# AngelAngelXie/Final-Project-Monte-Carlo-Path-Tracer-with-Microfacet-BSDF

Measured on AMD Instinct MI355X. Metric: Msamples/s (pixels x spp), chess scene 1920x1080, PSNR vs CPU, higher is better.
Workload: dtype f32

## Files before the change

### final-project-monte-carlo-path-tracer-with-microfacet-bsdf_amd/csrc/mcpt_frame.h

```cpp
#pragma once
#include "mcpt_host.h"
#include "mcpt_adaptive.h"
#include "mcpt_denoise.h"
#include "mcpt_temporal.h"

namespace mcpt {

constexpr int32_t kMaxAovSpp = 65536;

inline bool frame_ok(int W, int H) { return W > 0 && H > 0 && (uint64_t)W * H <= 0x7fffffffull / 8; }

enum : unsigned {
    kOneCallFrame = 1u,
    kOneRank = 2u,
    kDenoisedFrame = 4u,
    kOneSample = 8u
};

int check_frame_call(const char *name, const mcpt_camera &cam, const mcpt_params &p, unsigned forbid);

void fill_stats(mcpt_stats *stats, uint64_t samples, uint64_t traced_primary, int32_t n_dir, const Totals &rt, Clock::time_point t0);

struct FrameCall {
    mcpt_scene *sc;
    const mcpt_params &p;
    Clock::time_point t0;
    CameraConst cc;
    PixelSet ps;
    int begin(const mcpt_camera &cam) {
        HIP_TRY(hipSetDevice(sc->device));
        (void)hipGetLastError();
        t0 = Clock::now();
        cc = make_camera(cam);
        return MCPT_OK;
    }
    int pixels(int32_t spp, float spp_total, float *fb_dev, hipStream_t st) { return prepare_pixels(sc, cc, p, spp, spp_total, fb_dev, st, ps); }
    int end(mcpt_stats *stats, uint64_t samples, uint64_t traced_primary, const Totals &rt) const {
        if (stats) fill_stats(stats, samples, traced_primary, p.n_dir_sample, rt, t0);
        if (rt.overflow) return fail(MCPT_ERR_OVERFLOW, "some paths outran the clamp stack (raise params.max_depth)");
        return MCPT_OK;
    }
};

int aov_pass(mcpt_scene *sc, const CameraConst &cc, uint32_t seed, int32_t aov_spp, int32_t spec_depth, bool centre, float *aov_dev, hipStream_t st);
int check_features(const char *name, const mcpt_feature_opts *features, int32_t aov_spp, bool &centre);
int motion_pass(mcpt_scene *sc, const CameraConst &cc, const CameraConst &prev_cc, uint32_t seed, int32_t aov_spp, int32_t spec_depth, bool centre,
                float4 *maps, uint64_t map_rays, float *motion_dev, hipStream_t st);
uint64_t motion_map_rays(uint64_t n_px, int32_t aov_spp);

struct AdaptiveBufs {
    float *fb = nullptr;
    double *mom = nullptr;
    int32_t *spp = nullptr;
    float *err = nullptr;
    uint8_t *stamp = nullptr;
    const float *guide = nullptr;
    float guide_max_history = 0.f;
    uint32_t *list[2] = {nullptr, nullptr};
    int4 *cand[2] = {nullptr, nullptr};
    uint8_t *flags = nullptr;
    void *temp = nullptr;
// ... 59 lines not shown
```

### final-project-monte-carlo-path-tracer-with-microfacet-bsdf_amd/csrc/mcpt_host.h

```cpp
#pragma once
#include <hip/hip_runtime.h>

#include <algorithm>
#include <chrono>
#include <cstring>
#include <string>
#include <vector>

#include "mcpt_kernels.h"

namespace mcpt {

extern thread_local std::string g_err;

inline int fail(int code, const std::string &msg) {
    g_err = msg;
    return code;
}

#define HIP_TRY(expr)                                                                                   \
    do {                                                                                                \
        hipError_t e_ = (expr);                                                                         \
        if (e_ != hipSuccess)                                                                           \
            return fail(e_ == hipErrorOutOfMemory ? MCPT_ERR_OOM : MCPT_ERR_HIP,                        \
// ... 135 lines not shown
    DevBuf<int32_t> key_channel;
    int pix_key[5] = {0, 0, 0, 0, 0};
    uint32_t n_pix = 0;
};

struct Knobs {
    bool overlap = true;
    bool queue_ahead = true;
    bool timing = true;
    bool verbose = false;
    int pools = 1;
    int drain_batch = 4;
    uint64_t pool_min_work = 1ull << 20;
    uint32_t shadow_grid_per_cu = 128;
    uint32_t direct_grid_per_cu = 64;
    uint32_t ring_start = 0;
    int host_delay_us = 0;
    float halfspace_slack_scale = 1.f;
    float tir_bound_scale = 1.f;
    float cone_tol_scale = 1.f;
    float cull_rho_scale = 1.f;
    bool sky_cull = true;
    bool small_scene = true;
    uint64_t fake_free_mb = 0;
    void read();
};

enum KClass { K_CLOSEST = 0, K_SHADOW, K_SHADE, K_GENERATE, K_RESOLVE, K_DIRECT, K_NCLASS };

struct Timer {
    bool enabled = true;
    int bank = 0;
    std::vector<hipEvent_t> pool[2];
    struct Rec { int a, b, cls; };
    std::vector<Rec> recs[2];
    size_t used[2] = {0, 0};
    double ms[K_NCLASS] = {0, 0, 0, 0, 0, 0};
    uint64_t count[K_NCLASS] = {0, 0, 0, 0, 0, 0};
    Timer() = default;
    Timer(const Timer &) = delete;
    Timer &operator=(const Timer &) = delete;
    ~Timer() {
        for (int k = 0; k < 2; ++k)
            for (hipEvent_t e : pool[k]) (void)hipEventDestroy(e);
    }
    int get() {
// ... 16 lines not shown
        recs[bank].push_back({a, b, cls});
    }
    void collect_bank(int k) {
        for (const Rec &r : recs[k]) {
            float t = 0.f;
            if (hipEventElapsedTime(&t, pool[k][r.a], pool[k][r.b]) == hipSuccess) ms[r.cls] += t;
        }
        recs[k].clear();
        used[k] = 0;
    }
    void collect() {
        collect_bank(0);
        collect_bank(1);
    }
    void reset() {
        for (int i = 0; i < K_NCLASS; ++i) { ms[i] = 0; count[i] = 0; }
        for (int k = 0; k < 2; ++k) { recs[k].clear(); used[k] = 0; }
        bank = 0;
    }
};

struct Totals {
    uint64_t iterations = 0, shaded = 0, closest = 0, shadow = 0, direct = 0, pushes = 0, overflow = 0;
    double ms[K_NCLASS] = {0, 0, 0, 0, 0, 0};
    uint64_t cnt[K_NCLASS] = {0, 0, 0, 0, 0, 0};
    Totals &operator+=(const Totals &o) {
        iterations += o.iterations;
        shaded += o.shaded;
        closest += o.closest;
        shadow += o.shadow;
        direct += o.direct;
        pushes += o.pushes;
        overflow += o.overflow;
        for (int c = 0; c < K_NCLASS; ++c) {
            ms[c] += o.ms[c];
            cnt[c] += o.cnt[c];
        }
        return *this;
    }
};

struct GeomBufs {
    DevBuf<Node> nodes;
    DevBuf<QNode> qnodes;
    DevBuf<TriGeom> tri_geom;
    DevBuf<TriShade> tri_shade;
    DevBuf<SphereRec> spheres;
    DevBuf<mcpt_triangle> tris;
    DevBuf<LightRec> lights;
    DevBuf<LightNode> light_nodes;
    DevBuf<LightTri> light_tris;
    void swap_prims(GeomBufs &o) {
        nodes.swap(o.nodes);
        qnodes.swap(o.qnodes);
        tri_geom.swap(o.tri_geom);
        tri_shade.swap(o.tri_shade);
// ... 26 lines not shown
    BuildChoice choice;
};

struct alignas(16) MoveSeg {
    int32_t first_lane;
    int32_t count;
    int32_t first_tri;
    int32_t object;
    float m[12];
    float c0[3];
    int32_t raw;
};
static_assert(sizeof(MoveSeg) == 80, "MoveSeg must be 80 bytes");
void launch_move_objects(const MoveSeg *d_segs, int32_t n_segs, int32_t n_lanes, const mcpt_triangle *tris0, mcpt_triangle *tris_cur,
                         TriGeom *tri_geom, TriShade *tri_shade, SphereRec *spheres, hipStream_t s);

}

struct mcpt_scene {
    int device = 0;
    int device_sharers = 1;
    mcpt::Knobs knobs;
    mcpt_scene_info info{};
    mcpt::SceneMeta meta;
    mcpt::SceneSource src;
    mcpt::GeomBufs geom;
    mcpt::DevBuf<mcpt::TriGeom> snap_tri;
    mcpt::DevBuf<mcpt::SphereRec> snap_sph;
    bool has_snapshot = false;
    mcpt::DevBuf<mcpt_triangle> tris0;
    mcpt::DevBuf<int32_t> sphere_obj;
    mcpt::DevBuf<mcpt::MoveSeg> segs;
    mcpt::DevBuf<mcpt::MaterialRec> mats;
    mcpt::DevBuf<mcpt::InstRec> inst;
    mcpt::DevBuf<float> env;
    mcpt::DevBuf<unsigned long long> dbg;
    mcpt::DevScene view{};
    mcpt::Event fork;
    mcpt::SharedBufs shared;
    struct PoolCtx {
        mcpt::Stream main;
        mcpt::Stream side[2];
        mcpt::Event join[2];
        mcpt::Event book;
        mcpt::Event shaded, readback;
        int rc = 0;
// ... 67 lines not shown
```

### final-project-monte-carlo-path-tracer-with-microfacet-bsdf_amd/csrc/mcpt_kernels.h

```cpp
#pragma once
#include <hip/hip_runtime.h>

#include <cstddef>

#include "mcpt_device.h"

namespace mcpt {

constexpr uint32_t kFresh = 1u << 16;
constexpr uint32_t kTerminate = 1u << 17;
constexpr uint32_t kInside = 1u << 18;
constexpr uint32_t kPassBit = 1u << 20;
constexpr uint32_t kNoDirect = 1u << 19;

struct alignas(128) HotCounter {
    uint32_t v;
    uint32_t pad[31];
};
constexpr uint32_t kShadowShards = 32;
__host__ __device__ inline uint32_t shadow_region(uint32_t capacity) {
    return (((capacity + 63u) / 64u + kShadowShards - 1u) / kShadowShards) * 64u;
}
struct Counters {
    HotCounter n_paths[2];
    HotCounter n_rays[2];
    HotCounter n_direct[2];
    HotCounter free_head, free_tail;
    HotCounter n_prays[2];
    HotCounter live[2];
    HotCounter pushes;
    HotCounter overflow;
    HotCounter ended;
    unsigned long long tot_shaded, tot_direct, tot_shadow, tot_cont, tot_iterations, tot_pushes, tot_ended;
    uint32_t last_shadow;
    HotCounter n_shadow[2][kShadowShards];
    HotCounter n_shadow_w[2][kShadowShards];
};
constexpr size_t kCountersHeadBytes = offsetof(Counters, n_shadow);

struct Wave {
    uint4 *rec0;
    float4 *rec1;
    float4 *ray_o;
    float4 *ray_d;
    uint4 *hit;
    float *contrib;
    uint2 *fresh;
};

struct Scratch {
    float4 *vtx0;
    float4 *vtx1;
    float4 *vtx2;
    uint32_t *vtx_j;
    float4 *shq_o;
    float4 *shq_d;
};

constexpr int32_t kCandNone = 0x7fffffff;
constexpr int32_t kCandTraverse = 0x7ffffffe;

struct RenderConst {
    float rr_rate, inv_rr;
    int32_t n_dir, enable_shadow;
    uint32_t seed;
    int32_t mode;
    const uint32_t *pixel_list;
    const int4 *pixel_cand;
    int32_t s_pass[2], sample_offset[2];
    int32_t s_pass_shift[2];
    const uint32_t *key_pixel, *key_sample;
    const int32_t *key_channel;
    int32_t max_depth;
    int32_t track_live;
    uint32_t pool;
    float4 *stack;
    float *result[2];
    uint32_t *free_slots;
    uint32_t free_mask;
    uint32_t ray_cap;
    Counters *counters;
};

struct CameraConst {
    int32_t width, height, use_dof;
    float scale, aspect, focal_distance, aperture_radius;
    float eye[3];
    float orient[9];
};

constexpr int kSmallNodes = 64, kSmallTris = 64, kSmallSphereSlots = 16;
constexpr int kSmallMats = 12, kSmallLights = 4, kSmallLightNodes = 8, kSmallLightTris = 8;
constexpr int kSmallStk = 8;

struct RetryList {
    uint32_t *count;
    uint32_t *done;
// ... 57 lines not shown
```

### final-project-monte-carlo-path-tracer-with-microfacet-bsdf_amd/csrc/mcpt_kernels.hip

```cpp
#include <algorithm>
#include <cfloat>
#include <cstdlib>

#include "mcpt_kernels.h"
#include "mcpt_traverse.h"

namespace mcpt {

namespace {

#ifndef MCPT_SHADE_BLOCK
#define MCPT_SHADE_BLOCK 512
#endif
constexpr int kShadeBlock = MCPT_SHADE_BLOCK;

constexpr int kMaxAlloc = 9;
constexpr int kMaxWaves = 16;
struct BlockAllocShared {
    uint32_t cnt[kMaxWaves][kMaxAlloc];
    uint32_t base[kMaxAlloc];
};

template <int N>
MCPT_DI void block_alloc_begin(BlockAllocShared &sh, const bool (&want)[N], const uint32_t (&mult)[N], uint32_t *const (&counter)[N],
                               const bool (&subtract)[N], uint32_t (&prefix)[N]) {
    static_assert(N <= kMaxAlloc, "too many allocation requests");
    const uint32_t n_waves = blockDim.x >> 6;
    const uint32_t lane = lane_id();
    const uint32_t wave = threadIdx.x >> 6;
#pragma unroll
    for (int k = 0; k < N; ++k) {
        const unsigned long long mask = __ballot(want[k]);
        prefix[k] = __builtin_amdgcn_mbcnt_hi((uint32_t)(mask >> 32), __builtin_amdgcn_mbcnt_lo((uint32_t)mask, 0u));
        if (lane == 0) sh.cnt[wave][k] = (uint32_t)__popcll(mask);
    }
    __syncthreads();
#pragma unroll
    for (int k = 0; k < N; ++k) {
        if (threadIdx.x == (unsigned)k) {
// ... 504 lines not shown
    camera_ray_from<true>(cam, (int)(m % (uint32_t)cam.width), (int)(m / (uint32_t)cam.width), u, pos, dir);
    o[j] = make_float4(pos.x, pos.y, pos.z, 0.f);
    d[j] = make_float4(dir.x, dir.y, dir.z, 0.f);
}

__global__ __launch_bounds__(kBlock) void k_init_free(uint32_t *free_slots, Counters *c, uint32_t pool, uint32_t start, uint32_t mask) {
    const uint32_t j = blockIdx.x * kBlock + threadIdx.x;
    if (j < pool) free_slots[(start + j) & mask] = j;
    if (j == 0) {
        c->n_paths[0].v = c->n_paths[1].v = 0;
        c->n_rays[0].v = c->n_rays[1].v = 0;
        c->free_head.v = start;
        c->free_tail.v = start + pool;
        c->n_prays[0].v = c->n_prays[1].v = 0;
        c->live[0].v = c->live[1].v = 0;
        for (uint32_t k = 0; k < kShadowShards; ++k) {
            c->n_shadow[0][k].v = c->n_shadow[1][k].v = 0;
            c->n_shadow_w[0][k].v = c->n_shadow_w[1][k].v = 0;
        }
        c->n_direct[0].v = c->n_direct[1].v = 0;
        c->pushes.v = 0;
        c->overflow.v = 0;
        c->ended.v = 0;
        c->last_shadow = 0;
        c->tot_shaded = c->tot_direct = c->tot_shadow = c->tot_cont = c->tot_iterations = c->tot_pushes = c->tot_ended = 0;
    }
}

MCPT_DI bool sample_light(const DevScene &S, const float u[4], f3 &x_l, f3 &n_l, f3 &emit, float &pdf, int32_t &prim) {
    float area_sum = S.light_area_sum;
    const float p = u[0] * area_sum;
    area_sum = 0.f;
    for (int k = 0; k < S.n_lights; ++k) {
        const LightRec L = S.lights[k];
        area_sum += L.area;
        if (p <= area_sum) {
            const MaterialRec &m = S.mats[L.mat];
            if (L.kind == MCPT_OBJ_MESH) {
                float pp = sqrtf(u[1]) * L.root_area;
                int32_t ref = L.root;
                while (ref >= 0) {
                    const LightNode N = S.light_nodes[ref];
                    if (pp < N.left_area) {
                        ref = N.left;
                    } else {
                        pp = pp - N.left_area;
                        ref = N.right;
                    }
// ... 270 lines not shown
    const bool past_gate = false;
    const bool zero_direct = do_shade && direct_is_zero(S, m, q, n, wo, inside, ch, &by_tir);
#else
    const bool by_tir = false, past_gate = false;
    const bool zero_direct = do_shade && direct_is_zero(S, m, q, n, wo, inside, ch);
#endif
#if defined(MCPT_TRAVERSAL_STATS) || defined(MCPT_CHECK_DIRECT_SKIP)
    bool behind = false;
    if (do_shade && S.n_lights > 0) {
        const f3 L = mk3(S.light_center[0], S.light_center[1], S.light_center[2]) - q;
        behind = dot(L, L) > S.light_radius * S.light_radius * 1.0201f && emitters_behind(S, n, L);
    }
#else
    const bool behind = false;
#endif
#ifdef MCPT_CHECK_DIRECT_SKIP
    const bool need_direct = do_shade;
#else
    const bool need_direct = do_shade && !zero_direct;
#endif

    const bool ends_here = do_shade && !has_cont && !need_direct;
    const bool done = finished || ends_here;
    const bool want[9] = {done, do_shade && !ends_here, has_cont, need_direct, pushed, overflow, done && C.track_live && pq == 0,
                          done && C.track_live && pq == 1, ends_here};
    const uint32_t mult[9] = {1u, 1u, 1u, 1u, 1u, 1u, 1u, 1u, 1u};
    uint32_t *const ctr[9] = {&C.counters->free_tail.v, &C.counters->n_paths[next_idx].v, &C.counters->n_rays[next_idx].v,
                              &C.counters->n_direct[next_idx].v, &C.counters->pushes.v, &C.counters->overflow.v,
                              &C.counters->live[0].v, &C.counters->live[1].v, &C.counters->ended.v};
    const bool sub[9] = {false, false, false, false, false, false, true, true, false};
    uint32_t prefix[9], idx[9];
#ifdef MCPT_TRAVERSAL_STATS
    const long long tb0 = clock64();
#endif
    block_alloc_begin<9>(sh, want, mult, ctr, sub, prefix);
#ifdef MCPT_TRAVERSAL_STATS
    const long long tb1 = clock64();
#endif

    float kr = 0.f, ev = 0.f, aw = 0.f, pd = 0.f;
    f3 p2 = mk3(0, 0, 0), wi = mk3(0, 0, 1);
    if (do_shade) {
        const f3 mfn = mat_sample(m, n, u0[0], u0[1]);
        kr = mat_fresnel(m, rd, mfn, ch);
        const bool isReflect = u0[3] < kr;
        if (isReflect) p2 = (dot(wo, mfn) < 0) ? (p - n * kEps) : (p + n * kEps);
        else p2 = (dot(wo, mfn) < 0) ? (p + n * kEps) : (p - n * kEps);
        if (has_cont) {
            wi = isReflect ? mat_reflect(wo, mfn) : mat_refract(m, rd, mfn, ch);
            if (m.isDirac) {
                ev = mat_eval(m, wi, wo, n, ch, uv, isReflect);
                aw = -1.f;
            } else {
                aw = fabsf(dot(wo, n));
                mat_eval_pdf_rough(m, wi, wo, n, ch, uv, isReflect, ev, pd);
            }
        }
    }

#ifdef MCPT_TRAVERSAL_STATS
    const long long tb2 = clock64();
#endif
    block_alloc_end<9>(sh, mult, prefix, idx);
#ifdef MCPT_TRAVERSAL_STATS
    if (S.dbg && lane_id() == 0) {
        const long long tb3 = clock64();
        atomicAdd(&S.dbg[20], (unsigned long long)(tb1 - tb0));
        atomicAdd(&S.dbg[21], (unsigned long long)(tb3 - tb2));
        atomicAdd(&S.dbg[22], (unsigned long long)(tb3 - t_wave0));
        atomicAdd(&S.dbg[23], 1ull);
    }
    if (S.dbg) {
        int nd = 0;
        for (int t = 0; t < 4; ++t) nd += __ballot(do_shade && m.type == t) != 0ull ? 1 : 0;
        const unsigned long long ms = __ballot(do_shade);
        if (lane_id() == 0) {
            atomicAdd(&S.dbg[24 + nd], 1ull);
            atomicAdd(&S.dbg[29], (unsigned long long)__popcll(ms));
        }
    }
#endif
    if (done) C.free_slots[idx[0] & C.free_mask] = slot;
    if (!do_shade) return;
    if (ends_here) {
        const float l_dir = inside ? (float)((1. - (double)kr) * (double)0.f) : kr * 0.f;
        (pq ? C.result[1] : C.result[0])[pid] = unwind(C, slot, depth, l_dir);
        return;
    }
    const uint32_t j = idx[1], rj = idx[2], dj = idx[3];

    if (need_direct) {
        Xs.vtx0[dj] = make_float4(q.x, q.y, q.z, uv.x);
        Xs.vtx1[dj] = make_float4(n.x, n.y, n.z, uv.y);
        Xs.vtx2[dj] = make_float4(wo.x, wo.y, wo.z, __uint_as_float((uint32_t)mat_id | ((uint32_t)ch << 16) | (inside ? (1u << 18) : 0u) |
                                                                    (zero_direct ? (1u << 19) : 0u) | (behind ? (1u << 20) : 0u) | (by_tir ? (1u << 21) : 0u) |
                                                                    (past_gate ? (1u << 22) : 0u)));
        Xs.vtx_j[dj] = j;
    }
    uint32_t flags = depth | (inside ? kInside : 0u) | (need_direct ? 0u : kNoDirect) | (pq ? kPassBit : 0u);
    if (has_cont) {
        next.ray_o[rj] = make_float4(p2.x, p2.y, p2.z, 0.f);
        next.ray_d[rj] = make_float4(wi.x, wi.y, wi.z, 0.f);
    } else {
        flags |= kTerminate;
    }
    next.rec0[j] = make_uint4(pid, has_cont ? rj : slot, flags, __float_as_uint(kr));
    if (has_cont) next.rec1[j] = make_float4(ev, aw, pd, __uint_as_float(slot));
}

#ifndef MCPT_DIRECT_WAVES
#define MCPT_DIRECT_WAVES 7
#endif
template <bool SMALL>
__global__ __launch_bounds__(kBlock, MCPT_DIRECT_WAVES) void k_direct(DevScene S, RenderConst C, Wave next, Scratch Xs, int next_idx) {
    if constexpr (SMALL) {
        __shared__ SmallGeomLds small_geom;
        __shared__ SmallLightLds small_lights;
        stage_small_geom(S, small_geom);
        stage_small_lights(S, small_lights);
        __syncthreads();
    }
    const uint32_t n_dir = (uint32_t)C.n_dir;
    const uint32_t total = C.counters->n_direct[next_idx].v * n_dir;
    for (uint32_t base = blockIdx.x * kBlock; base < total; base += gridDim.x * kBlock) {
    const uint32_t g = base + threadIdx.x;
// ... 273 lines not shown
    uint32_t n_shadow = shard->v;
    shard->v = 0;
    for (int o = 32; o > 0; o >>= 1) n_shadow += (uint32_t)__shfl_xor((int)n_shadow, o);
    switch (threadIdx.x) {
    case 0: {
        c->tot_shadow += n_shadow;
        c->last_shadow = n_shadow;
        break;
    }
    case 1: c->tot_shaded += from_host ? n_next : c->n_paths[nxt].v; break;
    case 2: c->tot_cont += from_host ? n_cont : c->n_rays[nxt].v; break;
    case 3: c->tot_direct += from_host ? n_direct : c->n_direct[nxt].v; break;
    case 4: c->tot_iterations += 1; break;
    case 8: {
        const uint32_t v = c->ended.v;
        c->ended.v = 0;
        c->tot_ended += v;
        break;
    }
    case 9: {
        const uint32_t v = c->pushes.v;
        c->pushes.v = 0;
        c->tot_pushes += v;
        break;
    }
    case 5: c->n_paths[cur_idx].v = 0; break;
    case 6: c->n_rays[cur_idx].v = 0; break;
    case 10: c->n_prays[cur_idx].v = 0; break;
    case 7: c->n_direct[cur_idx].v = 0; break;
    default: break;
    }
}

void launch_bookkeep(Counters *c, int cur_idx, bool from_host, uint32_t n_next, uint32_t n_cont, uint32_t n_direct, hipStream_t s) {
    hipLaunchKernelGGL(k_bookkeep, dim3(1), dim3(64), 0, s, c, cur_idx, from_host ? 1 : 0, n_next, n_cont, n_direct);
}

void launch_init_free(uint32_t *free_slots, Counters *c, uint32_t pool, uint32_t start, uint32_t mask, hipStream_t s) {
    hipLaunchKernelGGL(k_init_free, dim3(blocks(pool)), dim3(kBlock), 0, s, free_slots, c, pool, start, mask);
}

constexpr uint32_t kRetraceGrid = 256;
#ifdef MCPT_LDS_ONLY_STACKS
#define MCPT_STACK_DISPATCH(height, KERNEL, RETRACE, ...)                                          \
    do {                                                                                           \
        if ((height) <= 17) hipLaunchKernelGGL((KERNEL<16, false, false>), __VA_ARGS__);           \
// ... 128 lines not shown
```

### final-project-monte-carlo-path-tracer-with-microfacet-bsdf_amd/csrc/mcpt_query.hip

```cpp
#include <cmath>

#include "mcpt_cull.h"
#include "mcpt_host.h"

using namespace mcpt;

namespace {

std::vector<float4> pack3(const float *v, size_t n) {
    std::vector<float4> out(n);
    for (size_t i = 0; i < n; ++i) out[i] = make_float4(v[3 * i], v[3 * i + 1], v[3 * i + 2], 0.f);
    return out;
}
void unpack3(const std::vector<float4> &v, float *out) {
    for (size_t i = 0; i < v.size(); ++i) {
        out[3 * i] = v[i].x;
        out[3 * i + 1] = v[i].y;
        out[3 * i + 2] = v[i].z;
    }
}

}

extern "C" {
// ... 40 lines not shown
    const int64_t chunk_max = 1 << 20;
    ctx.timer.reset();
    ctx.timer.enabled = false;
    for (int64_t base = 0; base < n; base += chunk_max) {
        const uint32_t m = (uint32_t)std::min<int64_t>(chunk_max, n - base);
        const uint32_t pool = std::max<uint32_t>((m + 2) / 3 * 3, 3 * 256);
        HIP_TRY(ensure_workspace(ctx, std::max(pool, w.pool), p.n_dir_sample, std::max(max_depth, w.max_depth), stack_uses_retry(sc->view.height)));
        HIP_TRY(sh.result.alloc(m));
        HIP_TRY(upload(w.wave[0].ray_o, pack3(origins + 3 * base, m)));
        HIP_TRY(upload(w.wave[0].ray_d, pack3(dirs + 3 * base, m)));
        HIP_TRY(upload(sh.key_pixel, pixel + base, m));
        HIP_TRY(upload(sh.key_sample, sample + base, m));
        HIP_TRY(upload(sh.key_channel, channel + base, m));
        RenderConst C = base_consts(p, w.max_depth);
        C.mode = 1;
        C.key_pixel = sh.key_pixel.p;
        C.key_sample = sh.key_sample.p;
        C.key_channel = sh.key_channel.p;
        C.result[0] = C.result[1] = sh.result.p;
        Totals tot;
        const std::vector<PassPlan> plan{PassPlan{0u, m, 1, 0}};
        const int rc = drained(run_wavefront(sc, ctx, C, nullptr, plan, nullptr, nullptr, tot));
        if (rc != MCPT_OK) return rc;
        HIP_TRY(download(out + base, sh.result, m));
    }
    return MCPT_OK;
}

int mcpt_camera_rays(mcpt_scene *sc, const mcpt_camera *cam, uint32_t seed, int64_t n, const uint32_t *pixel,
                     const uint32_t *sample, float *origins, float *dirs) {
    if (!sc || !cam || n < 0 || (n > 0 && (!pixel || !sample || !origins || !dirs))) return fail(MCPT_ERR_ARG, "mcpt_camera_rays: bad argument");
    if (n == 0) return MCPT_OK;
    if (n > 0x7fffffff) return fail(MCPT_ERR_ARG, "mcpt_camera_rays: too many rays for one call");
    HIP_TRY(hipSetDevice(sc->device));
    DevBuf<uint32_t> dP, dS;
    DevBuf<float4> dO, dD;
    HIP_TRY(dO.alloc(n));
    HIP_TRY(dD.alloc(n));
    HIP_TRY(upload(dP, pixel, n));
    HIP_TRY(upload(dS, sample, n));
    launch_camera_rays(make_camera(*cam), seed, (uint32_t)n, dP.p, dS.p, dO.p, dD.p, nullptr);
    std::vector<float4> o(n), d(n);
    HIP_TRY(download(o.data(), dO, n));
    HIP_TRY(download(d.data(), dD, n));
    unpack3(o, origins);
    unpack3(d, dirs);
// ... 211 lines not shown
```

### final-project-monte-carlo-path-tracer-with-microfacet-bsdf_amd/csrc/mcpt_upload.hip

```cpp
#include <cmath>
#include <cstdio>
#include <cstdlib>
#include <memory>
#include <thread>

#include "mcpt_host.h"
#include "mcpt_lbvh.h"
#include "mcpt_move.h"

using namespace mcpt;

thread_local std::string mcpt::g_err;

void Knobs::read() {
    auto off = [](const char *n) { const char *v = std::getenv(n); return v && v[0] == '0'; };
    overlap = !off("MCPT_OVERLAP");
    queue_ahead = !off("MCPT_QUEUE_AHEAD");
    timing = !off("MCPT_TIMING");
    verbose = std::getenv("MCPT_RENDER_VERBOSE") != nullptr;
    sky_cull = !off("MCPT_SKY_CULL");
    small_scene = !off("MCPT_SMALL_SCENE");
    const char *v;
    if ((v = std::getenv("MCPT_POOLS"))) pools = (v[0] == '2') ? 2 : 1;
    if ((v = std::getenv("MCPT_DRAIN_BATCH"))) drain_batch = std::max(1, std::atoi(v));
    if ((v = std::getenv("MCPT_POOL_MIN_WORK"))) pool_min_work = (uint64_t)std::max(1, std::atoi(v));
    if ((v = std::getenv("MCPT_SHADOW_GRID_PER_CU"))) shadow_grid_per_cu = (uint32_t)std::max(1, std::atoi(v));
    if ((v = std::getenv("MCPT_DIRECT_GRID_PER_CU"))) direct_grid_per_cu = (uint32_t)std::max(0, std::atoi(v));
#ifdef MCPT_TEST_HOOKS
    if ((v = std::getenv("MCPT_RING_START"))) ring_start = (uint32_t)std::strtoul(v, nullptr, 0);
    if ((v = std::getenv("MCPT_HOST_DELAY_US"))) host_delay_us = std::atoi(v);
    if ((v = std::getenv("MCPT_HALFSPACE_SLACK_SCALE"))) halfspace_slack_scale = (float)std::atof(v);
    if ((v = std::getenv("MCPT_TIR_BOUND_SCALE"))) tir_bound_scale = (float)std::atof(v);
    if ((v = std::getenv("MCPT_CONE_TOL_SCALE"))) cone_tol_scale = (float)std::atof(v);
    if ((v = std::getenv("MCPT_CULL_RHO_SCALE"))) cull_rho_scale = (float)std::atof(v);
    if ((v = std::getenv("MCPT_FAKE_FREE_MB"))) fake_free_mb = (uint64_t)std::max(1, std::atoi(v));
#endif
}

double mcpt::warm_up_device(int device) {
    const auto t0 = Clock::now();
    if (hipSetDevice(device) != hipSuccess) return 0.0;
    uint32_t *p = nullptr;
    if (hipMalloc((void **)&p, 256) == hipSuccess) {
        launch_add_frame(reinterpret_cast<float *>(p), reinterpret_cast<float *>(p), 0u, nullptr);
// ... 565 lines not shown
            for (int c = 0; c < 3; ++c) inst_shift[3 * k + c] = I[k].shift[c];
            inst_root_first[2 * k] = I[k].root;
            inst_root_first[2 * k + 1] = I[k].first_tri;
        }
    }
    for (int k = 0; k < 3; ++k) {
        info->root_min[k] = v.root_min[k];
        info->root_max[k] = v.root_max[k];
        info->q_origin[k] = v.q_origin[k];
        info->q_cell[k] = v.q_cell[k];
    }
    if (!boxes || !children || info->n_nodes == 0) return MCPT_OK;
    std::vector<Node> nodes((size_t)info->n_nodes);
    HIP_TRY(download(nodes.data(), sc->geom.nodes, nodes.size()));
    std::vector<QNode> qn;
    if (qboxes && info->quantised) {
        qn.resize(nodes.size());
        HIP_TRY(download(qn.data(), sc->geom.qnodes, qn.size()));
    }
    export_nodes(info->n_nodes, nodes.data(), qn.empty() ? nullptr : qn.data(), boxes, children, qboxes);
    return MCPT_OK;
}

int mcpt_scene_get_info(const mcpt_scene *sc, mcpt_scene_info *info) {
    if (!sc || !info) return fail(MCPT_ERR_ARG, "mcpt_scene_get_info: null argument");
    *info = sc->info;
    return MCPT_OK;
}

}
```

### final-project-monte-carlo-path-tracer-with-microfacet-bsdf_amd/csrc/mcpt_wavefront.hip

```cpp
#include <unistd.h>

#include <cmath>
#include <cstdio>
#include <thread>

#include "mcpt_host.h"
#include "mcpt_cull.h"

namespace mcpt {

hipError_t ensure_workspace(PoolCtx &ctx, uint32_t pool, int32_t n_dir, int32_t max_depth, bool retry_lists) {
    Workspace &w = ctx.ws;
    hipError_t e;
    const size_t n_rays = (size_t)pool + pool / 3 + 64;
    for (int k = 0; k < 2; ++k) {
        WaveBufs &b = w.wave[k];
        if ((e = b.rec0.alloc(pool)) != hipSuccess) return e;
        if ((e = b.rec1.alloc(pool)) != hipSuccess) return e;
        if ((e = b.ray_o.alloc(n_rays)) != hipSuccess) return e;
        if ((e = b.ray_d.alloc(n_rays)) != hipSuccess) return e;
        if ((e = b.hit.alloc(n_rays)) != hipSuccess) return e;
        if ((e = b.contrib.alloc((size_t)pool * n_dir)) != hipSuccess) return e;
        if ((e = b.fresh.alloc(pool / 3 + 64)) != hipSuccess) return e;
    }
// ... 70 lines not shown
            for (int by = y0; by < y1; by += 8)
                for (int bx = x0; bx < x1; bx += 8)
                    for (int y = by; y < std::min(y1, by + 8); ++y)
                        for (int x = bx; x < std::min(x1, bx + 8); ++x) out.push_back((uint32_t)(y * W + x));
        }
}

int run_wavefront(mcpt_scene *sc, PoolCtx &ctx, const RenderConst &C0, const CameraConst *cam, const std::vector<PassPlan> &plan,
                  const AccumPlan *acc, hipStream_t st, Totals &tot) {
    Workspace &w = ctx.ws;
    Timer &T = ctx.timer;
    RenderConst C = C0;
    C.pool = w.pool;
    C.stack = w.stack.p;
    C.free_slots = w.free_slots.p;
    C.free_mask = w.free_ring - 1u;
    C.ray_cap = w.ray_cap;
    C.counters = w.counters.p;
    const uint32_t pool = w.pool;
    const int n_dir = C.n_dir;
    const int P = (int)plan.size();
    C.track_live = (acc && P > 1) ? 1 : 0;
    const Knobs &K = sc->knobs;
    launch_init_free(w.free_slots.p, w.counters.p, pool, K.ring_start, w.free_ring - 1u, st);
    if (ctx.side[1].s) {
        HIP_TRY(hipEventRecord(ctx.book, st));
        for (int k = 0; k < 2; ++k) HIP_TRY(hipStreamWaitEvent(ctx.side[k], ctx.book, 0));
    }
    int cur = 0;
    uint32_t n_cur_max = 0;
    int issue_pass = 0, accum_next = 0;
    uint32_t issued = 0;
    uint32_t free_known = 0;
    bool have_counters = false;
    double cont_ratio = 1.0, direct_ratio = 1.0;
    double shadow_ratio = 1.0;
    uint32_t n_direct_prev = 0, n_direct_prev2 = 0;
    bool n_cur_exact = false;
    long it = 0;
    std::vector<long> issue_done_iter(P, -1);
    hipStream_t s_close = ctx.side[0].s ? ctx.side[0].s : st, s_prim = ctx.side[1].s ? ctx.side[1].s : st;

    auto set_pass_consts = [&](int pi) {
        const int32_t sp = plan[pi].s_pass;
        C.s_pass[pi & 1] = sp;
        C.sample_offset[pi & 1] = plan[pi].sample_offset;
// ... 140 lines not shown
        free_known = w.h_counters->free_tail.v - w.h_counters->free_head.v;
        if (n_cur_max > 0) {
            if (n_cur_exact) {
                cont_ratio = (double)n_cont / n_cur_max;
                direct_ratio = (double)n_direct / n_cur_max;
            }
            if (n_direct_prev2 > 0) shadow_ratio = std::min(1.0, (double)w.h_counters->last_shadow / ((double)n_direct_prev2 * n_dir));
        }
        n_direct_prev2 = n_direct_prev;
        n_direct_prev = n_direct;
        n_cur_max = n_next;
        n_cur_exact = true;
        cur = nxt;
    }
    HIP_TRY(hipMemcpyAsync(w.h_counters.p, w.counters.p, sizeof(Counters), hipMemcpyDeviceToHost, st));
    HIP_TRY(hipStreamSynchronize(st));
    T.collect();
    const Counters &hc = *w.h_counters.p;
    tot.pushes += hc.tot_pushes + hc.pushes.v;
    tot.overflow += hc.overflow.v;
    tot.iterations += hc.tot_iterations;
    tot.shaded += hc.tot_shaded + hc.tot_ended + hc.ended.v;
    tot.direct += hc.tot_direct;
    tot.closest += hc.tot_cont;
    tot.shadow += hc.tot_shadow;
    for (uint32_t k = 0; k < kShadowShards; ++k) tot.shadow += hc.n_shadow[0][k].v + hc.n_shadow[1][k].v + hc.n_shadow_w[0][k].v + hc.n_shadow_w[1][k].v;
    return MCPT_OK;
}

int drained(int rc) {
    if (rc != MCPT_OK) {
        const std::string keep = g_err;
        (void)hipDeviceSynchronize();
        (void)hipGetLastError();
        g_err = keep;
    }
    return rc;
}

static uint64_t bytes_per_pool_path(int n_dir, int max_depth) {
    const double rays = 1.0 + 1.0 / 3.0;
    const double wave = 16 + 16 + rays * 48 + 4.0 * n_dir + 8.0 / 3.0;
    const double scratch = 3 * 16 + 4 + 32.0 * n_dir;
    const double retrace = 4.0 * (rays + n_dir + 1.0 / 3.0);
    return (uint64_t)(2 * wave + scratch + retrace + 16.0 * max_depth + 16.0);
}

// ... 135 lines not shown
                    return;
                }
                c1.rc = run_wavefront(sc, c1, C, &cc, plan1, nullptr, c1.main, tot[1]);
                if (c1.rc != MCPT_OK) c1.err = g_err;
            });
            const int rc0 = run_wavefront(sc, sc->pools[0], C, &cc, plan0, nullptr, st, tot[0]);
            worker.join();
            if (rc0 != MCPT_OK) return drained(rc0);
            if (c1.rc != MCPT_OK) return drained(fail(c1.rc, c1.err));
            Timer &T0 = sc->pools[0].timer;
            T0.timed(K_RESOLVE, st, [&] { launch_accumulate(C.result[0], pixel_list, n_pix, s_now, spp_total, fb_dev, moments, st); });
        }
    }
    HIP_TRY(hipStreamSynchronize(st));
    sc->pools[0].timer.collect();
    HIP_TRY(hipGetLastError());
    for (int k = 0; k < n_pools; ++k) {
        for (int c = 0; c < K_NCLASS; ++c) {
            tot[k].ms[c] = sc->pools[k].timer.ms[c];
            tot[k].cnt[c] = sc->pools[k].timer.count[c];
        }
        rt += tot[k];
    }
    return MCPT_OK;
}

}
```

### final-project-monte-carlo-path-tracer-with-microfacet-bsdf_amd/hip_backend.py

```python
from __future__ import annotations

import ctypes as C
import os

import numpy as np

HERE = os.path.dirname(os.path.abspath(__file__))
LIB_PATH = os.environ.get("MCPT_LIB") or os.path.join(HERE, "libmcpt_hip.so")
CHECK_LIB_PATH = os.path.join(HERE, "libmcpt_hip_check.so")

EXPORTS = ["mcpt_scene_create", "mcpt_scene_destroy", "mcpt_render", "mcpt_render_device", "mcpt_render_adaptive", "mcpt_render_aovs",
           "mcpt_render_aovs_ex", "mcpt_denoise", "mcpt_render_denoised", "mcpt_intersect",
           "mcpt_cast_rays", "mcpt_camera_rays", "mcpt_scene_get_info", "mcpt_bvh_dump", "mcpt_scene_create_ex", "mcpt_scene_dump_bvh", "mcpt_tonemap", "mcpt_tonemap_device", "mcpt_debug_fmath", "mcpt_debug_material", "mcpt_debug_scene", "mcpt_debug_shadow", "mcpt_debug_counters",
           "mcpt_cull_bound", "mcpt_debug_classify",
           "mcpt_scene_update", "mcpt_group_update", "mcpt_transform_triangles",
           "mcpt_scene_snapshot", "mcpt_render_motion", "mcpt_temporal_blend", "mcpt_temporal_accumulate",
           "mcpt_temporal_accumulate_ex",
           "mcpt_sequence_create", "mcpt_sequence_frame", "mcpt_sequence_reset", "mcpt_sequence_destroy",
           "mcpt_sequence_create_ex", "mcpt_sequence_flags",
           "mcpt_temporal_history_len", "mcpt_render_adaptive_guided", "mcpt_render_adaptive_denoised",
           "mcpt_sequence_create_adaptive", "mcpt_sequence_counts",
           "mcpt_render_motion_ex", "mcpt_sequence_create_motion",
           "mcpt_temporal_accumulate_weighted", "mcpt_temporal_history_weight", "mcpt_render_adaptive_weighted",
           "mcpt_sequence_create_weighted", "mcpt_sequence_weight",
           "mcpt_temporal_accumulate_moments", "mcpt_moments_variance", "mcpt_sequence_create_moments", "mcpt_sequence_moments",
           "mcpt_centre_rays", "mcpt_render_aovs_features", "mcpt_render_motion_features", "mcpt_sequence_create_features",
           "mcpt_denoise_feedback", "mcpt_sequence_create_feedback", "mcpt_sequence_history",
           "mcpt_group_create", "mcpt_group_render", "mcpt_group_size", "mcpt_group_get_info", "mcpt_group_scene", "mcpt_group_destroy", "mcpt_group_last_error",
           "mcpt_last_error", "mcpt_version"]


class McptError(RuntimeError):
    def __init__(self, code, msg):
        super().__init__("mcpt error %d: %s" % (code, msg))
        self.code = code


class SceneDesc(C.Structure):
    _fields_ = [("n_objects", C.c_int32), ("n_triangles", C.c_int32), ("n_materials", C.c_int32),
                ("env_w", C.c_int32), ("env_h", C.c_int32), ("background", C.c_float * 3),
                ("objects", C.c_void_p), ("triangles", C.c_void_p), ("materials", C.c_void_p), ("env_pixels", C.c_void_p)]


class Params(C.Structure):
    _fields_ = [("spp", C.c_int32), ("spp_total", C.c_int32), ("sample_offset", C.c_int32), ("rr_rate", C.c_float),
                ("n_dir_sample", C.c_int32), ("enable_shadow", C.c_int32), ("seed", C.c_uint32), ("accumulate", C.c_int32),
                ("tile_size", C.c_int32), ("rank", C.c_int32), ("nranks", C.c_int32), ("spp_per_pass", C.c_int32),
                ("pool_paths", C.c_int32), ("max_depth", C.c_int32)]


# ... 172 lines not shown

def lib(path=None):
    path = path or LIB_PATH
    if path not in _libs:
        if not os.path.exists(path):
            raise FileNotFoundError("%s is missing: build it with `python __graft_entry__.py` (hipcc, gfx950)" % path)
        L = C.CDLL(path)
        L.mcpt_last_error.restype = C.c_char_p
        L.mcpt_version.restype = C.c_char_p
        L.mcpt_scene_create.restype = C.c_int
        L.mcpt_scene_create.argtypes = [C.POINTER(SceneDesc), C.c_int, C.POINTER(C.c_void_p)]
        L.mcpt_scene_create_ex.restype = C.c_int
        L.mcpt_scene_create_ex.argtypes = [C.POINTER(SceneDesc), C.c_int, C.c_void_p, C.POINTER(C.c_void_p)]
        L.mcpt_scene_dump_bvh.restype = C.c_int
        L.mcpt_scene_dump_bvh.argtypes = [C.c_void_p, C.POINTER(BvhInfo), C.c_void_p, C.c_void_p, C.c_void_p, C.c_void_p, C.c_void_p]
        L.mcpt_tonemap.restype = C.c_int
        L.mcpt_tonemap.argtypes = [C.c_void_p, C.c_void_p, C.c_int64, C.c_void_p]
        L.mcpt_tonemap_device.restype = C.c_int
        L.mcpt_tonemap_device.argtypes = [C.c_void_p, C.c_void_p, C.c_int64, C.c_void_p, C.c_void_p]
        L.mcpt_scene_destroy.restype = None
        L.mcpt_scene_destroy.argtypes = [C.c_void_p]
        L.mcpt_scene_get_info.restype = C.c_int
        L.mcpt_scene_get_info.argtypes = [C.c_void_p, C.POINTER(SceneInfo)]
        L.mcpt_bvh_dump.restype = C.c_int
        L.mcpt_bvh_dump.argtypes = [C.POINTER(SceneDesc), C.POINTER(BvhInfo), C.c_void_p, C.c_void_p, C.c_void_p, C.c_void_p, C.c_void_p]
        L.mcpt_render.restype = C.c_int
        L.mcpt_render.argtypes = [C.c_void_p, C.c_void_p, C.POINTER(Params), C.c_void_p, C.POINTER(Stats)]
        L.mcpt_render_adaptive.restype = C.c_int
        L.mcpt_render_adaptive.argtypes = [C.c_void_p, C.c_void_p, C.POINTER(Params), C.POINTER(Adaptive), C.c_void_p, C.c_void_p, C.c_void_p,
                                           C.POINTER(AdaptiveInfo), C.POINTER(Stats)]
        L.mcpt_render_aovs.restype = C.c_int
        L.mcpt_render_aovs.argtypes = [C.c_void_p, C.c_void_p, C.c_uint32, C.c_int32, C.c_void_p]
        L.mcpt_render_aovs_ex.restype = C.c_int
        L.mcpt_render_aovs_ex.argtypes = [C.c_void_p, C.c_void_p, C.c_uint32, C.c_int32, C.c_int32, C.c_void_p]
        L.mcpt_denoise.restype = C.c_int
        L.mcpt_denoise.argtypes = [C.c_void_p, C.c_int32, C.c_int32, C.c_void_p, C.c_void_p, C.c_void_p, C.POINTER(DenoiseOpts), C.c_void_p]
        L.mcpt_render_denoised.restype = C.c_int
        L.mcpt_render_denoised.argtypes = [C.c_void_p, C.c_void_p, C.POINTER(Params), C.POINTER(DenoiseOpts), C.c_void_p, C.c_void_p, C.c_void_p,
                                           C.c_void_p, C.POINTER(DenoiseInfo), C.POINTER(Stats)]
        L.mcpt_scene_snapshot.restype = C.c_int
        L.mcpt_scene_snapshot.argtypes = [C.c_void_p]
        L.mcpt_render_motion.restype = C.c_int
        L.mcpt_render_motion.argtypes = [C.c_void_p, C.c_void_p, C.c_void_p, C.c_uint32, C.c_int32, C.c_void_p]
        L.mcpt_render_motion_ex.restype = C.c_int
        L.mcpt_render_motion_ex.argtypes = [C.c_void_p, C.c_void_p, C.c_void_p, C.c_uint32, C.c_int32, C.c_int32, C.c_void_p]
        L.mcpt_sequence_create_motion.restype = C.c_int
# ... 235 lines not shown

    def tonemap(self, fb):
        fb = np.ascontiguousarray(fb, dtype=np.float32)
        out = np.zeros(fb.shape[:-1] + (4,), dtype=np.uint8)
        _check(self.L.mcpt_tonemap(self.h, _ptr(fb), fb.size // 3, _ptr(out)), L=self.L)
        return out

    def debug_counters(self):
        out = np.zeros(16, dtype=np.uint64)
        _check(self.L.mcpt_debug_counters(self.h, _ptr(out)), L=self.L)
        return out

    def __del__(self):
        try:
            self.close()
        except Exception:
            pass

    def info(self):
        i = SceneInfo()
        _check(self.L.mcpt_scene_get_info(self.h, C.byref(i)), L=self.L)
        return {k: getattr(i, k) for k, _ in i._fields_}

    def params(self, spp=None, seed=1, spp_total=0, sample_offset=0, accumulate=0, tile_size=32, rank=0, nranks=1,
               n_dir_sample=None, spp_per_pass=0, pool_paths=0, max_depth=0):
        sd = self.sd
        return Params(spp=int(spp if spp is not None else sd.spp), spp_total=int(spp_total), sample_offset=int(sample_offset),
                      rr_rate=float(sd.rr_rate), n_dir_sample=int(n_dir_sample if n_dir_sample is not None else sd.n_dir_sample),
                      enable_shadow=int(sd.enable_shadow), seed=int(seed), accumulate=int(accumulate), tile_size=int(tile_size),
                      rank=int(rank), nranks=int(nranks), spp_per_pass=int(spp_per_pass), pool_paths=int(pool_paths),
                      max_depth=int(max_depth))

    def render(self, camera=None, fb=None, **kw):
        cam = np.ascontiguousarray(camera if camera is not None else self.sd.camera)
        W, H = int(cam["width"].reshape(-1)[0]), int(cam["height"].reshape(-1)[0])
        if fb is None:
            fb = np.zeros((H, W, 3), dtype=np.float32)
        p = self.params(**kw)
        st = Stats()
        _check(self.L.mcpt_render(self.h, _ptr(cam), C.byref(p), _ptr(fb), C.byref(st)), L=self.L)
        return fb, st

    def render_adaptive(self, min_spp, threshold, rel_floor=1e-3, dilate=1, camera=None, **kw):
        cam = np.ascontiguousarray(camera if camera is not None else self.sd.camera)
        W, H = int(cam["width"].reshape(-1)[0]), int(cam["height"].reshape(-1)[0])
        fb = np.zeros((H, W, 3), dtype=np.float32)
# ... 594 lines not shown
```

### include/mcpt.h

```cpp
#ifndef MCPT_H
#define MCPT_H

#include <stdint.h>

#ifdef __cplusplus
extern "C" {
#endif

typedef enum {
    MCPT_OK = 0,
    MCPT_ERR_ARG = 1,
    MCPT_ERR_HIP = 2,
    MCPT_ERR_OOM = 3,
    MCPT_ERR_LIMIT = 4,
    MCPT_ERR_OVERFLOW = 5
} mcpt_status;

enum { MCPT_SMOOTH_CONDUCTOR = 0, MCPT_ROUGH_CONDUCTOR = 1, MCPT_SMOOTH_DIELECTRIC = 2, MCPT_ROUGH_DIELECTRIC = 3 };
enum { MCPT_OBJ_MESH = 0, MCPT_OBJ_SPHERE = 1 };

typedef struct {
    float v0[3], v1[3], v2[3];
    float t0[2], t1[2], t2[2];
} mcpt_triangle;
// ... 334 lines not shown
    int32_t n_devices;
    int32_t uses_rccl;
    double build_ms, upload_ms_max, init_ms_max, setup_ms;
} mcpt_group_info;
int mcpt_group_get_info(const mcpt_group *group, mcpt_group_info *info);
mcpt_scene *mcpt_group_scene(mcpt_group *group, int index);
int mcpt_group_update(mcpt_group *group, int32_t n, const mcpt_object_transform *moves);
void mcpt_group_destroy(mcpt_group *group);
const char *mcpt_group_last_error(void);

typedef struct {
    int32_t n_nodes, bvh_height, n_lights, n_prims;
    uint64_t scene_bytes;
    double build_ms;
    double upload_ms;
    int32_t builder;
    int32_t quantised;
    int32_t n_instances;
    int32_t lds_resident;
    double init_ms;
} mcpt_scene_info;
int mcpt_scene_get_info(const mcpt_scene *scene, mcpt_scene_info *info);

typedef struct {
    int32_t n_nodes, root, stack_entries, quantised;
    float root_min[3], root_max[3];
    float q_origin[3], q_cell[3];
    int32_t n_instances, n_leaf_prims;
} mcpt_bvh_info;
int mcpt_bvh_dump(const mcpt_scene_desc *desc, mcpt_bvh_info *info, float *boxes, int32_t *children, uint16_t *qboxes,
                  float *inst_shift, int32_t *inst_root_first);
int mcpt_scene_dump_bvh(mcpt_scene *scene, mcpt_bvh_info *info, float *boxes, int32_t *children, uint16_t *qboxes,
                        float *inst_shift, int32_t *inst_root_first);

int mcpt_debug_fmath(mcpt_scene *scene, int kind, int64_t n, const float *x, const float *y, float *out);

int mcpt_debug_material(mcpt_scene *scene, int kind, int64_t n, const float *in, const int32_t *sel, float *out);

int mcpt_debug_scene(mcpt_scene *scene, int kind, int64_t n, const float *in, float *out);

int mcpt_debug_shadow(mcpt_scene *scene, int32_t list, int64_t n, const float *origins, const float *dirs, const float *dist,
                      const uint8_t *found, const int32_t *shard , uint8_t *visible);

typedef struct {
    int32_t classified;
    float rho, scale, aspect, focal, lens;
// ... 17 lines not shown
```

Measured before the change: 5611.

## Share continuation rays among adjacent lanes with identical smooth-conductor rays

In the shade kernel, lanes whose continuation comes from a smooth conductor compare their source ray index with the two lanes below them. When it matches, they reuse the leader's slot in the next ray buffer instead of allocating and writing their own, so duplicate mirror continuations are traced once. The aim is to cut closest-hit traversal work when several paths share the same deterministic reflection. It adds shuffles, a tenth block-allocation counter, and a host-side API and counters for traced versus shared rays. It is on by default and can be disabled with MCPT_SHARE_RAYS.

```diff
diff --git a/final-project-monte-carlo-path-tracer-with-microfacet-bsdf_amd/csrc/mcpt_frame.h b/final-project-monte-carlo-path-tracer-with-microfacet-bsdf_amd/csrc/mcpt_frame.h
--- a/final-project-monte-carlo-path-tracer-with-microfacet-bsdf_amd/csrc/mcpt_frame.h
+++ b/final-project-monte-carlo-path-tracer-with-microfacet-bsdf_amd/csrc/mcpt_frame.h
@@ -37,6 +37,8 @@
     int pixels(int32_t spp, float spp_total, float *fb_dev, hipStream_t st) { return prepare_pixels(sc, cc, p, spp, spp_total, fb_dev, st, ps); }
     int end(mcpt_stats *stats, uint64_t samples, uint64_t traced_primary, const Totals &rt) const {
         if (stats) fill_stats(stats, samples, traced_primary, p.n_dir_sample, rt, t0);
+        sc->last_cont_traced = rt.cont_traced;
+        sc->last_cont_shared = rt.cont_shared;
         if (rt.overflow) return fail(MCPT_ERR_OVERFLOW, "some paths outran the clamp stack (raise params.max_depth)");
         return MCPT_OK;
     }
diff --git a/final-project-monte-carlo-path-tracer-with-microfacet-bsdf_amd/csrc/mcpt_host.h b/final-project-monte-carlo-path-tracer-with-microfacet-bsdf_amd/csrc/mcpt_host.h
--- a/final-project-monte-carlo-path-tracer-with-microfacet-bsdf_amd/csrc/mcpt_host.h
+++ b/final-project-monte-carlo-path-tracer-with-microfacet-bsdf_amd/csrc/mcpt_host.h
@@ -181,6 +181,7 @@
     float cull_rho_scale = 1.f;
     bool sky_cull = true;
     bool small_scene = true;
+    bool share_rays = true;
     uint64_t fake_free_mb = 0;
     void read();
 };
@@ -243,6 +244,7 @@
 
 struct Totals {
     uint64_t iterations = 0, shaded = 0, closest = 0, shadow = 0, direct = 0, pushes = 0, overflow = 0;
+    uint64_t cont_traced = 0, cont_shared = 0;
     double ms[K_NCLASS] = {0, 0, 0, 0, 0, 0};
     uint64_t cnt[K_NCLASS] = {0, 0, 0, 0, 0, 0};
     Totals &operator+=(const Totals &o) {
@@ -253,6 +255,8 @@
         direct += o.direct;
         pushes += o.pushes;
         overflow += o.overflow;
+        cont_traced += o.cont_traced;
+        cont_shared += o.cont_shared;
         for (int c = 0; c < K_NCLASS; ++c) {
             ms[c] += o.ms[c];
             cnt[c] += o.cnt[c];
@@ -325,6 +329,7 @@
     int device_sharers = 1;
     mcpt::Knobs knobs;
     mcpt_scene_info info{};
+    uint64_t last_cont_traced = 0, last_cont_shared = 0;
     mcpt::SceneMeta meta;
     mcpt::SceneSource src;
     mcpt::GeomBufs geom;
diff --git a/final-project-monte-carlo-path-tracer-with-microfacet-bsdf_amd/csrc/mcpt_kernels.h b/final-project-monte-carlo-path-tracer-with-microfacet-bsdf_amd/csrc/mcpt_kernels.h
--- a/final-project-monte-carlo-path-tracer-with-microfacet-bsdf_amd/csrc/mcpt_kernels.h
+++ b/final-project-monte-carlo-path-tracer-with-microfacet-bsdf_amd/csrc/mcpt_kernels.h
@@ -31,7 +31,8 @@
     HotCounter pushes;
     HotCounter overflow;
     HotCounter ended;
-    unsigned long long tot_shaded, tot_direct, tot_shadow, tot_cont, tot_iterations, tot_pushes, tot_ended;
+    HotCounter shared;
+    unsigned long long tot_shaded, tot_direct, tot_shadow, tot_cont, tot_iterations, tot_pushes, tot_ended, tot_shared;
     uint32_t last_shadow;
     HotCounter n_shadow[2][kShadowShards];
     HotCounter n_shadow_w[2][kShadowShards];
@@ -73,6 +74,7 @@
     const int32_t *key_channel;
     int32_t max_depth;
     int32_t track_live;
+    int32_t share_rays;
     uint32_t pool;
     float4 *stack;
     float *result[2];
diff --git a/final-project-monte-carlo-path-tracer-with-microfacet-bsdf_amd/csrc/mcpt_kernels.hip b/final-project-monte-carlo-path-tracer-with-microfacet-bsdf_amd/csrc/mcpt_kernels.hip
--- a/final-project-monte-carlo-path-tracer-with-microfacet-bsdf_amd/csrc/mcpt_kernels.hip
+++ b/final-project-monte-carlo-path-tracer-with-microfacet-bsdf_amd/csrc/mcpt_kernels.hip
@@ -14,7 +14,7 @@
 #endif
 constexpr int kShadeBlock = MCPT_SHADE_BLOCK;
 
-constexpr int kMaxAlloc = 9;
+constexpr int kMaxAlloc = 10;
 constexpr int kMaxWaves = 16;
 struct BlockAllocShared {
     uint32_t cnt[kMaxWaves][kMaxAlloc];
@@ -565,8 +565,9 @@
         c->pushes.v = 0;
         c->overflow.v = 0;
         c->ended.v = 0;
+        c->shared.v = 0;
         c->last_shadow = 0;
-        c->tot_shaded = c->tot_direct = c->tot_shadow = c->tot_cont = c->tot_iterations = c->tot_pushes = c->tot_ended = 0;
+        c->tot_shaded = c->tot_direct = c->tot_shadow = c->tot_cont = c->tot_iterations = c->tot_pushes = c->tot_ended = c->tot_shared = 0;
     }
 }
 
@@ -883,18 +884,25 @@
 
     const bool ends_here = do_shade && !has_cont && !need_direct;
     const bool done = finished || ends_here;
-    const bool want[9] = {done, do_shade && !ends_here, has_cont, need_direct, pushed, overflow, done && C.track_live && pq == 0,
-                          done && C.track_live && pq == 1, ends_here};
-    const uint32_t mult[9] = {1u, 1u, 1u, 1u, 1u, 1u, 1u, 1u, 1u};
-    uint32_t *const ctr[9] = {&C.counters->free_tail.v, &C.counters->n_paths[next_idx].v, &C.counters->n_rays[next_idx].v,
-                              &C.counters->n_direct[next_idx].v, &C.counters->pushes.v, &C.counters->overflow.v,
-                              &C.counters->live[0].v, &C.counters->live[1].v, &C.counters->ended.v};
-    const bool sub[9] = {false, false, false, false, false, false, true, true, false};
-    uint32_t prefix[9], idx[9];
+    uint32_t lead = 0;
+    {
+        const bool cand = has_cont && C.share_rays && m.type == MCPT_SMOOTH_CONDUCTOR;
+        const uint32_t mine = cand ? ray_idx : 0xffffffffu;
+        const uint32_t up1 = (uint32_t)__shfl_up((int)mine, 1), up2 = (uint32_t)__shfl_up((int)mine, 2);
+        if (cand) lead = (lane_id() >= 2u && up2 == mine) ? 2u : ((lane_id() >= 1u && up1 == mine) ? 1u : 0u);
+    }
+    const bool want[10] = {done, do_shade && !ends_here, has_cont && lead == 0u, need_direct, pushed, overflow, done && C.track_live && pq == 0,
+                           done && C.track_live && pq == 1, ends_here, lead != 0u};
+    const uint32_t mult[10] = {1u, 1u, 1u, 1u, 1u, 1u, 1u, 1u, 1u, 1u};
+    uint32_t *const ctr[10] = {&C.counters->free_tail.v, &C.counters->n_paths[next_idx].v, &C.counters->n_rays[next_idx].v,
+                               &C.counters->n_direct[next_idx].v, &C.counters->pushes.v, &C.counters->overflow.v,
+                               &C.counters->live[0].v, &C.counters->live[1].v, &C.counters->ended.v, &C.counters->shared.v};
+    const bool sub[10] = {false, false, false, false, false, false, true, true, false, false};
+    uint32_t prefix[10], idx[10];
 #ifdef MCPT_TRAVERSAL_STATS
     const long long tb0 = clock64();
 #endif
-    block_alloc_begin<9>(sh, want, mult, ctr, sub, prefix);
+    block_alloc_begin<10>(sh, want, mult, ctr, sub, prefix);
 #ifdef MCPT_TRAVERSAL_STATS
     const long long tb1 = clock64();
 #endif
@@ -922,7 +930,8 @@
 #ifdef MCPT_TRAVERSAL_STATS
     const long long tb2 = clock64();
 #endif
-    block_alloc_end<9>(sh, mult, prefix, idx);
+    block_alloc_end<10>(sh, mult, prefix, idx);
+    const uint32_t rj = (uint32_t)__shfl((int)idx[2], (int)(lane_id() - lead));
 #ifdef MCPT_TRAVERSAL_STATS
     if (S.dbg && lane_id() == 0) {
         const long long tb3 = clock64();
@@ -948,7 +957,7 @@
         (pq ? C.result[1] : C.result[0])[pid] = unwind(C, slot, depth, l_dir);
         return;
     }
-    const uint32_t j = idx[1], rj = idx[2], dj = idx[3];
+    const uint32_t j = idx[1], dj = idx[3];
 
     if (need_direct) {
         Xs.vtx0[dj] = make_float4(q.x, q.y, q.z, uv.x);
@@ -960,8 +969,10 @@
     }
     uint32_t flags = depth | (inside ? kInside : 0u) | (need_direct ? 0u : kNoDirect) | (pq ? kPassBit : 0u);
     if (has_cont) {
-        next.ray_o[rj] = make_float4(p2.x, p2.y, p2.z, 0.f);
-        next.ray_d[rj] = make_float4(wi.x, wi.y, wi.z, 0.f);
+        if (lead == 0u) {
+            next.ray_o[rj] = make_float4(p2.x, p2.y, p2.z, 0.f);
+            next.ray_d[rj] = make_float4(wi.x, wi.y, wi.z, 0.f);
+        }
     } else {
         flags |= kTerminate;
     }
@@ -1281,6 +1292,12 @@
         const uint32_t v = c->pushes.v;
         c->pushes.v = 0;
         c->tot_pushes += v;
+        break;
+    }
+    case 11: {
+        const uint32_t v = c->shared.v;
+        c->shared.v = 0;
+        c->tot_shared += v;
         break;
     }
     case 5: c->n_paths[cur_idx].v = 0; break;
diff --git a/final-project-monte-carlo-path-tracer-with-microfacet-bsdf_amd/csrc/mcpt_query.hip b/final-project-monte-carlo-path-tracer-with-microfacet-bsdf_amd/csrc/mcpt_query.hip
--- a/final-project-monte-carlo-path-tracer-with-microfacet-bsdf_amd/csrc/mcpt_query.hip
+++ b/final-project-monte-carlo-path-tracer-with-microfacet-bsdf_amd/csrc/mcpt_query.hip
@@ -86,6 +86,9 @@
         const std::vector<PassPlan> plan{PassPlan{0u, m, 1, 0}};
         const int rc = drained(run_wavefront(sc, ctx, C, nullptr, plan, nullptr, nullptr, tot));
         if (rc != MCPT_OK) return rc;
+        if (base == 0) sc->last_cont_traced = sc->last_cont_shared = 0;
+        sc->last_cont_traced += tot.cont_traced;
+        sc->last_cont_shared += tot.cont_shared;
         HIP_TRY(download(out + base, sh.result, m));
     }
     return MCPT_OK;
diff --git a/final-project-monte-carlo-path-tracer-with-microfacet-bsdf_amd/csrc/mcpt_upload.hip b/final-project-monte-carlo-path-tracer-with-microfacet-bsdf_amd/csrc/mcpt_upload.hip
--- a/final-project-monte-carlo-path-tracer-with-microfacet-bsdf_amd/csrc/mcpt_upload.hip
+++ b/final-project-monte-carlo-path-tracer-with-microfacet-bsdf_amd/csrc/mcpt_upload.hip
@@ -20,6 +20,7 @@
     verbose = std::getenv("MCPT_RENDER_VERBOSE") != nullptr;
     sky_cull = !off("MCPT_SKY_CULL");
     small_scene = !off("MCPT_SMALL_SCENE");
+    share_rays = !off("MCPT_SHARE_RAYS");
     const char *v;
     if ((v = std::getenv("MCPT_POOLS"))) pools = (v[0] == '2') ? 2 : 1;
     if ((v = std::getenv("MCPT_DRAIN_BATCH"))) drain_batch = std::max(1, std::atoi(v));
@@ -631,6 +632,13 @@
     return MCPT_OK;
 }
 
+int mcpt_scene_ray_counts(const mcpt_scene *sc, uint64_t *traced, uint64_t *shared) {
+    if (!sc || !traced || !shared) return fail(MCPT_ERR_ARG, "mcpt_scene_ray_counts: null argument");
+    *traced = sc->last_cont_traced;
+    *shared = sc->last_cont_shared;
+    return MCPT_OK;
+}
+
 int mcpt_scene_get_info(const mcpt_scene *sc, mcpt_scene_info *info) {
     if (!sc || !info) return fail(MCPT_ERR_ARG, "mcpt_scene_get_info: null argument");
     *info = sc->info;
diff --git a/final-project-monte-carlo-path-tracer-with-microfacet-bsdf_amd/csrc/mcpt_wavefront.hip b/final-project-monte-carlo-path-tracer-with-microfacet-bsdf_amd/csrc/mcpt_wavefront.hip
--- a/final-project-monte-carlo-path-tracer-with-microfacet-bsdf_amd/csrc/mcpt_wavefront.hip
+++ b/final-project-monte-carlo-path-tracer-with-microfacet-bsdf_amd/csrc/mcpt_wavefront.hip
@@ -116,6 +116,7 @@
     const int P = (int)plan.size();
     C.track_live = (acc && P > 1) ? 1 : 0;
     const Knobs &K = sc->knobs;
+    C.share_rays = K.share_rays ? 1 : 0;
     launch_init_free(w.free_slots.p, w.counters.p, pool, K.ring_start, w.free_ring - 1u, st);
     if (ctx.side[1].s) {
         HIP_TRY(hipEventRecord(ctx.book, st));
@@ -302,7 +303,10 @@
     tot.iterations += hc.tot_iterations;
     tot.shaded += hc.tot_shaded + hc.tot_ended + hc.ended.v;
     tot.direct += hc.tot_direct;
-    tot.closest += hc.tot_cont;
+    const uint64_t shared = hc.tot_shared + hc.shared.v;
+    tot.closest += hc.tot_cont + shared;
+    tot.cont_traced += hc.tot_cont;
+    tot.cont_shared += shared;
     tot.shadow += hc.tot_shadow;
     for (uint32_t k = 0; k < kShadowShards; ++k) tot.shadow += hc.n_shadow[0][k].v + hc.n_shadow[1][k].v + hc.n_shadow_w[0][k].v + hc.n_shadow_w[1][k].v;
     return MCPT_OK;
@@ -484,6 +488,14 @@
         }
         rt += tot[k];
     }
+    if (sc->knobs.verbose) {
+        uint64_t traced = 0, shared = 0;
+        for (int k = 0; k < n_pools; ++k) {
+            traced += tot[k].cont_traced;
+            shared += tot[k].cont_shared;
+        }
+        std::fprintf(stderr, "[mcpt render] continuation rays: %llu traced, %llu shared with a sibling's\n", (unsigned long long)traced, (unsigned long long)shared);
+    }
     return MCPT_OK;
 }
 
diff --git a/final-project-monte-carlo-path-tracer-with-microfacet-bsdf_amd/hip_backend.py b/final-project-monte-carlo-path-tracer-with-microfacet-bsdf_amd/hip_backend.py
--- a/final-project-monte-carlo-path-tracer-with-microfacet-bsdf_amd/hip_backend.py
+++ b/final-project-monte-carlo-path-tracer-with-microfacet-bsdf_amd/hip_backend.py
@@ -26,6 +26,7 @@
            "mcpt_temporal_accumulate_moments", "mcpt_moments_variance", "mcpt_sequence_create_moments", "mcpt_sequence_moments",
            "mcpt_centre_rays", "mcpt_render_aovs_features", "mcpt_render_motion_features", "mcpt_sequence_create_features",
            "mcpt_denoise_feedback", "mcpt_sequence_create_feedback", "mcpt_sequence_history",
+           "mcpt_scene_ray_counts",
            "mcpt_group_create", "mcpt_group_render", "mcpt_group_size", "mcpt_group_get_info", "mcpt_group_scene", "mcpt_group_destroy", "mcpt_group_last_error",
            "mcpt_last_error", "mcpt_version"]
 
@@ -244,6 +245,8 @@
         L.mcpt_scene_destroy.argtypes = [C.c_void_p]
         L.mcpt_scene_get_info.restype = C.c_int
         L.mcpt_scene_get_info.argtypes = [C.c_void_p, C.POINTER(SceneInfo)]
+        L.mcpt_scene_ray_counts.restype = C.c_int
+        L.mcpt_scene_ray_counts.argtypes = [C.c_void_p, C.POINTER(C.c_uint64), C.POINTER(C.c_uint64)]
         L.mcpt_bvh_dump.restype = C.c_int
         L.mcpt_bvh_dump.argtypes = [C.POINTER(SceneDesc), C.POINTER(BvhInfo), C.c_void_p, C.c_void_p, C.c_void_p, C.c_void_p, C.c_void_p]
         L.mcpt_render.restype = C.c_int
@@ -525,6 +528,11 @@
         _check(self.L.mcpt_scene_get_info(self.h, C.byref(i)), L=self.L)
         return {k: getattr(i, k) for k, _ in i._fields_}
 
+    def ray_counts(self):
+        t, s = C.c_uint64(0), C.c_uint64(0)
+        _check(self.L.mcpt_scene_ray_counts(self.h, C.byref(t), C.byref(s)), L=self.L)
+        return int(t.value), int(s.value)
+
     def params(self, spp=None, seed=1, spp_total=0, sample_offset=0, accumulate=0, tile_size=32, rank=0, nranks=1,
                n_dir_sample=None, spp_per_pass=0, pool_paths=0, max_depth=0):
         sd = self.sd
diff --git a/include/mcpt.h b/include/mcpt.h
--- a/include/mcpt.h
+++ b/include/mcpt.h
@@ -380,6 +380,8 @@
 } mcpt_scene_info;
 int mcpt_scene_get_info(const mcpt_scene *scene, mcpt_scene_info *info);
 
+int mcpt_scene_ray_counts(const mcpt_scene *scene, uint64_t *traced, uint64_t *shared);
+
 typedef struct {
     int32_t n_nodes, root, stack_entries, quantised;
     float root_min[3], root_max[3];
```

New measurement: 5768, median of 6. 2.8% higher.
